# googlegenomics/spark-examples

Hardware: AMD Instinct MI355X
Metric: variants/sec into N×N Gram + PCoA wall-clock, 2504 samples, 1/2/4/8 GPU (higher is better)
Workload: dtype fp4(e2m1)->f32->i32

## Files before the change

spark-examples_amd/csrc/operand.hip:

```cpp
#include <algorithm>
#include <cstring>

#include "pcoa_ctx.h"

using namespace pcoa;

namespace pcoa {

int fold_now(pcoa_ctx* c) {
  const int64_t count = (int64_t)s_count(c);
  if (!c->s64) {
    if (c->s64_spare) {
      c->s64 = c->s64_spare;
      c->s64_spare = nullptr;
    } else {
      HIP_TRY(c, dev_alloc((void**)&c->s64, sizeof(int64_t) * (size_t)count, c->device));
    }
    HIP_TRY(c, hipMemsetAsync(c->s64, 0, sizeof(int64_t) * (size_t)count, c->stream));
  }
  if (!c->is_strip) HIP_TRY(c, launch_symmetrize_i32(c->s32, c->n, c->stream));
  HIP_TRY(c, launch_fold_i32_to_i64(c->s32, c->s64, count, c->stream));
  c->variants_in_s32 = 0;
  c->dirty = false;
  return PCOA_OK;
// ... 8 lines not shown
  return rc;
}

int narrow_s64(pcoa_ctx* c) {
  if (!c->s64 || debug_knobs().no_narrow) return PCOA_OK;
  const int64_t count = (int64_t)s_count(c);
  if (!c->narrow_flag) HIP_TRY(c, dev_alloc((void**)&c->narrow_flag, 16, c->device));
  HIP_TRY(c, hipMemsetAsync(c->narrow_flag, 0, 16, c->stream));
  HIP_TRY(c, launch_narrow_i64_to_i32(c->s64, c->s32, count, c->narrow_flag, c->stream));
  HIP_TRY(c, hipMemcpyAsync(c->hw->coll, c->narrow_flag, 16, hipMemcpyDeviceToHost, c->stream));
  HIP_TRY(c, hipStreamSynchronize(c->stream));
  const int32_t overflow = (int32_t)(c->hw->coll[0] & 0xffffffff);
  const int64_t maxabs = c->hw->coll[1];
  if (overflow) {
    HIP_TRY(c, hipMemsetAsync(c->s32, 0, sizeof(int32_t) * (size_t)count, c->stream));
    return PCOA_OK;
  }
  if ((size_t)count * sizeof(int64_t) <= ((size_t)1 << 30)) {
    c->s64_spare = c->s64;
  } else {
    dev_free(c->s64);
  }
  c->s64 = nullptr;
  c->variants_in_s32 = maxabs;
  c->narrowed += 1;
  return PCOA_OK;
}

void account_gram(pcoa_ctx* c, int64_t cur, int64_t weight) {
  c->gram_launches += 1;
  c->gram_variants += cur;
  c->gram_flops += 2.0 * (double)cur * (double)c->n * (double)c->n;
  c->gram_bytes += 4.0 * (double)cur * (double)c->n + 4.0 * (double)c->n * (double)c->n;
  c->variants_in_s32 += cur * weight;
  c->dirty = true;
  c->strip_centering_set = false;
}

int fold_if_needed(pcoa_ctx* c, int64_t cur) {
  if (c->variants_in_s32 + cur > c->fold_threshold) {
    int rc = fp4_quiesce(c);
    if (rc != PCOA_OK) return rc;
    ScopedTimer t(c, T_FINALIZE);
    return fold_now(c);
  }
  return PCOA_OK;
}

static int64_t fp4_kb_bytes(const pcoa_ctx* c) { return gram_packed_npad(c->n) * (c->op_fmt == 2 ? 4 : 16); }
int64_t kb_of(const pcoa_ctx* c, int64_t nv) {
  const int64_t kb = (nv + 31) / 32;
  return c->op_fmt == 2 ? round_up(kb, 4) : kb;
}
static hipError_t launch_pack_operand(const pcoa_ctx* c, const void* x, int is_u8, int64_t ld, int64_t nv, int8_t* dst, int32_t* flag,
                               hipStream_t s, int64_t kb, int ring_wgs = 0) {
  if (ring_wgs > 0 && c->op_fmt == 2 && !is_u8)
    return launch_pack_kbits_ring(static_cast<const float*>(x), ld, nv, c->n, dst, flag, s, kb / 4, ring_wgs,
                                  8 + 1000 * std::max(0, debug_knobs().kbits_ring_prio));
  if (ring_wgs > 0 && c->op_fmt == 2 && is_u8)
    return launch_pack_kbits_ring_u8(static_cast<const uint8_t*>(x), ld, nv, c->n, dst, flag, s, kb / 4, ring_wgs, 8);
  return c->op_fmt == 2 ? launch_pack_kbits(x, is_u8, ld, nv, c->n, dst, flag, s, kb / 4)
                        : launch_pack_fp4(x, is_u8, ld, nv, c->n, dst, flag, s, kb);
}
static hipError_t launch_bits_operand(const pcoa_ctx* c, const uint32_t* bits, int64_t ld_words, int64_t nv, int8_t* dst, hipStream_t s,
                               int64_t kb) {
  return c->op_fmt == 2 ? launch_transpose_bits_kbits(bits, ld_words, nv, c->n, dst, s, kb / 4)
                        : launch_expand_bits_fp4(bits, ld_words, nv, c->n, dst, s, kb);
}
hipError_t launch_csr_operand(const pcoa_ctx* c, const int32_t* idx, const int64_t* offs, int64_t nv, int64_t offs_base,
                              int8_t* dst, hipStream_t s, int64_t kb) {
  return c->op_fmt == 2 ? launch_densify_csr_kbits(idx, offs, nv, offs_base, dst, c->n, c->err_flag, s, kb / 4)
                        : launch_densify_csr_fp4(idx, offs, nv, offs_base, dst, c->n, c->err_flag, s, kb);
}
static int32_t* fb_flag(pcoa_ctx* c, int b) { return c->fb_flags + 16 * b; }

int64_t fp4_target_kb(const pcoa_ctx* c) {
  const int64_t per_kb = fp4_kb_bytes(c);
  const int64_t by_launch = (c->fb_count == 2) ? kPipeVariants : kBatchVariants;
  return std::max<int64_t>(1, std::min(std::min(c->max_launch, by_launch) / 32, kBatchBytes / per_kb));
}

static int fork_to(pcoa_ctx* c, hipStream_t side) {
  if (side == c->stream) return PCOA_OK;
  if (debug_knobs().fork_lazy != 0) {
    if (hipStreamQuery(c->stream) == hipSuccess) return PCOA_OK;
    (void)hipGetLastError();
  }
  HIP_TRY(c, hipEventRecord(c->ev_fork, c->stream));
  HIP_TRY(c, hipStreamWaitEvent(side, c->ev_fork, 0));
  return PCOA_OK;
}

static int int8_chunk(pcoa_ctx* c, const void* x_chunk, int is_u8, int64_t cur, int64_t ld) {
  int rc = PCOA_OK;
  if ((rc = fp4_quiesce(c)) != PCOA_OK) return rc;
  const int64_t need = (int64_t)gram_packed_workspace_bytes(c->n, cur);
  if ((rc = ensure(c, &c->pack_buf, &c->pack_cap, need)) != PCOA_OK) return rc;
  HIP_TRY(c, hipMemsetAsync(c->err_flag + 1, 0, sizeof(int32_t), c->stream));
  {
    ScopedTimer t(c, T_PACK);
    hipError_t e = is_u8 ? launch_pack_u8_i8(static_cast<const uint8_t*>(x_chunk), ld, cur, c->n, c->pack_buf,
                                             c->err_flag, c->stream)
                         : launch_pack_f32_i8(static_cast<const float*>(x_chunk), ld, cur, c->n, c->pack_buf,
                                              c->err_flag, c->stream);
    if (e != hipSuccess) return hip_fail(c, e, "pack(i8) kernel launch");
    c->pack_launches += 1;
    c->pack_bytes += (is_u8 ? 1.0 : 4.0) * (double)cur * (double)c->n + (double)need;
  }
  HIP_TRY(c, hipMemcpyAsync(&c->hw->mmax, c->err_flag + 1, sizeof(int32_t), hipMemcpyDeviceToHost, c->stream));
  HIP_TRY(c, hipStreamSynchronize(c->stream));
  const int32_t mmax = c->hw->mmax;
// ... 16 lines not shown
}

int fp4_setup(pcoa_ctx* c) {
  if (c->fb_flags) return PCOA_OK;
  HIP_TRY(c, dev_alloc((void**)&c->fb_flags, 256, c->device));
  HIP_TRY(c, hipMemsetAsync(c->fb_flags, 0, 256, c->stream));
  HIP_TRY(c, hipHostMalloc((void**)&c->fb_flags_host, 256, hipHostMallocDefault));
  std::memset(c->fb_flags_host, 0, 256);
  HIP_TRY(c, hipEventCreateWithFlags(&c->ev_fork, hipEventDisableTiming));
  for (auto& b : c->fb) {
    HIP_TRY(c, hipEventCreateWithFlags(&b.packed, hipEventDisableTiming));
    HIP_TRY(c, hipEventCreateWithFlags(&b.consumed, hipEventDisableTiming));
  }
  const DebugKnobs& k = debug_knobs();
  const int ls = gram_lockstep_splitk(c->n, c->num_cu);
  c->lockstep_ok = !c->is_strip && ls > 0 && gram_lockstep_workgroups(c->n, ls) * 5 >= c->num_cu * 4;
  if (k.lockstep == 0) c->lockstep_ok = false;
  if (k.lockstep == 1) c->lockstep_ok = !c->is_strip && ls > 0;
  {
    const int64_t ntile = gram_packed_npad(c->n) / 256;
    const int64_t ntri = c->is_strip ? ntile * ((c->s_cols + 255) / 256 + 1) : ntile * (ntile + 1) / 2;
    c->kbits_mode = (ntri <= 4 * (int64_t)c->num_cu) ? 4 : 0;
    if (k.kbits_mode == 0 || k.kbits_mode == 4) c->kbits_mode = k.kbits_mode;
    if (k.kbits_mode == 5 && c->kbits_mode == 4) c->kbits_mode = 5;
    if (k.kbits_mode == 2 && !c->is_strip && ls > 0) c->kbits_mode = 2;
  }
  const int half = c->num_cu / 2;
  const int lsh = gram_lockstep_splitk(c->n, half);
  bool want = !c->is_strip && c->num_cu >= 64 && lsh > 0 && gram_packed_npad(c->n) >= 5 * 256;
  const int64_t cores_max = k.kbits_coreside_max_npad > 0 ? k.kbits_coreside_max_npad : kCoresideMaxNpad;
  const bool cores_shape = !c->is_strip && c->num_cu >= 64 && c->op_fmt == 2 && k.kbits_coreside != 0 &&
                           gram_packed_npad(c->n) >= 5 * 256 && gram_packed_npad(c->n) <= cores_max;
  want = want || cores_shape;
  if (k.pipeline == 0) want = false;
  if (k.pipeline == 1) want = !c->is_strip && (lsh > 0 || cores_shape);
  if (c->flags & PCOA_FLAG_NO_PIPELINE) want = false;
  if (want) {
    hipError_t e1 = hipStreamCreateWithFlags(&c->pack_stream, hipStreamNonBlocking);
    hipError_t e2 = (e1 == hipSuccess) ? hipStreamCreateWithFlags(&c->gram_stream, hipStreamNonBlocking) : e1;
    if (e1 == hipSuccess && e2 == hipSuccess) {
      c->pipe_ok = true;
      c->pipe_gram_cus = half;
      if (c->op_fmt == 2 && k.kbits_pipe_wgs >= 8 && k.kbits_pipe_wgs <= c->num_cu) c->pipe_gram_cus = k.kbits_pipe_wgs / 8 * 8;
      c->fb_count = 2;
      if (c->op_fmt == 2 && k.kbits_coreside != 0) {
        c->coreside = true;
        c->coreside_mode = (ls > 0 && gram_lockstep_workgroups(c->n, ls) * 5 >= c->num_cu * 4 && k.kbits_mode != 4) ? 2 : c->kbits_mode;
        if (k.kbits_mode == 2 && ls > 0) c->coreside_mode = 2;
        c->pipe_gram_cus = c->num_cu;
        if (k.kbits_pipe_wgs >= 8 && k.kbits_pipe_wgs <= c->num_cu) {
          c->pipe_gram_cus = k.kbits_pipe_wgs / 8 * 8;
          c->coreside_mode = 4;
        }
        c->ring_wgs = (k.kbits_ring_wgs > 0) ? k.kbits_ring_wgs : 2 * c->num_cu;
      }
    } else {
      (void)hipGetLastError();
      if (c->pack_stream) (void)hipStreamDestroy(c->pack_stream);
      c->pack_stream = c->gram_stream = nullptr;
    }
  }
  if (c->op_fmt == 2 && c->kbits_mode != 0) c->fb_count = 2;
  if (!c->pipe_ok && c->lockstep_ok) c->fb_count = 2;
  return PCOA_OK;
}

static int fp4_launch(pcoa_ctx* c, int bi, bool overlapped, int side_kind = 1) {
  pcoa_ctx::Fp4Buf& b = c->fb[bi];
  int rc = (bi == c->fb_active && !c->csr_pending.empty()) ? csr_validate(c) : PCOA_OK;
  if (rc != PCOA_OK) return rc;
  if (b.kb == 0) return PCOA_OK;
  rc = fold_if_needed(c, b.vars);
  if (rc != PCOA_OK) return rc;
  const int64_t per_kb = fp4_kb_bytes(c);
  const int64_t kb_pad = round_up(b.kb, 24);
  const bool side = overlapped && c->pipe_ok;
  hipStream_t gs = side ? c->gram_stream : c->stream;
  if (kb_pad > b.kb)
    HIP_TRY(c, hipMemsetAsync(b.p + b.kb * per_kb, 0, (size_t)((kb_pad - b.kb) * per_kb), b.fill_stream));
  if (gs != b.fill_stream) {
    HIP_TRY(c, hipEventRecord(b.packed, b.fill_stream));
    HIP_TRY(c, hipStreamWaitEvent(gs, b.packed, 0));
  }
  if ((rc = fork_to(c, gs)) != PCOA_OK) return rc;
  const int cus = side ? c->pipe_gram_cus : c->num_cu;
  const int32_t* skip = b.verify ? fb_flag(c, bi) : nullptr;
  {
    ScopedTimer t(c, T_GRAM, gs);
    hipError_t e = hipErrorInvalidValue;
    if (c->op_fmt == 2) {
      const int mode = !side ? c->kbits_mode : !c->coreside ? 4 : (side_kind == 3 ? c->kbits_mode : c->coreside_mode);
      const int w4 = debug_knobs().kbits_w4;
      const bool use_w4 = w4 != 0 && (!(side && c->coreside) || w4 == 2);
      auto launch = [&](int m) {
        return use_w4 ? launch_gram_kbits_w4(b.p, b.kb * 32, c->n, c->s32, cus, gs, m, skip, strip_of(c), debug_knobs().kbits_w4_diag)
                      : launch_gram_kbits(b.p, b.kb * 32, c->n, c->s32, cus, gs, m, skip, strip_of(c));
      };
      e = launch(mode);
      if (e != hipSuccess && mode != 0) {
        (void)hipGetLastError();
        e = launch(0);
      } else if (e == hipSuccess) {
        if (mode == 2) c->lockstep_launches += 1;
        if (mode == 4 || mode == 5) c->evensplit_launches += 1;
        if (side) c->pipeline_launches += 1;
      }
    } else {
// ... 39 lines not shown
    HIP_TRY(c, hipMemsetAsync(fb_flag(c, bi), 0, sizeof(int32_t), c->stream));
    if (redo) {
      c->fp4_fallbacks += (int64_t)b.chunks.size();
      c->i8_streak = 8;
      std::vector<pcoa_ctx::Fp4Chunk> chunks;
      chunks.swap(b.chunks);
      for (const auto& ch : chunks)
        if ((rc = int8_chunk(c, ch.x, ch.is_u8, ch.nv, ch.ld)) != PCOA_OK) break;
    }
  }
  b.chunks.clear();
  return rc;
}

int fp4_quiesce(pcoa_ctx* c) {
  int rc = c->csr_pending.empty() ? PCOA_OK : csr_validate(c);
  for (int bi = 0; bi < 2 && rc == PCOA_OK; ++bi) rc = fp4_resolve(c, bi);
  if (rc != PCOA_OK) return rc;
  for (auto& b : c->fb)
    if (b.kb > 0 && b.fill_stream && b.fill_stream != c->stream) HIP_TRY(c, hipStreamSynchronize(b.fill_stream));
  return PCOA_OK;
}

int fp4_flush(pcoa_ctx* c) {
  int rc = PCOA_OK;
  for (int bi = 0; bi < 2; ++bi)
    if (c->fb[bi].kb > 0 && (rc = fp4_launch(c, bi, false)) != PCOA_OK) return rc;
  return fp4_quiesce(c);
}

int fp4_sync_point(pcoa_ctx* c) {
  int rc = PCOA_OK;
  for (int bi = 0; bi < 2; ++bi)
    if (c->fb[bi].kb > 0 && c->fb[bi].verify && (rc = fp4_launch(c, bi, false)) != PCOA_OK) return rc;
  return fp4_quiesce(c);
}

int fp4_discard(pcoa_ctx* c) {
  if (!c->csr_pending.empty()) {
    const int rc = staging_wait_all(c, c->cs);
    if (rc != PCOA_OK) return rc;
    c->csr_pending.clear();
    if (c->csr_flag) HIP_TRY(c, hipMemsetAsync(c->csr_flag, 0, 16, c->stream));
  }
  for (int bi = 0; bi < 2; ++bi) {
    pcoa_ctx::Fp4Buf& b = c->fb[bi];
    int rc = fp4_resolve(c, bi, false);
    if (rc != PCOA_OK) return rc;
    if (b.kb > 0 && b.fill_stream && b.fill_stream != c->stream) HIP_TRY(c, hipStreamSynchronize(b.fill_stream));
    b.kb = 0;
    b.vars = 0;
    b.chunks.clear();
  }
  return PCOA_OK;
}

int fp4_grow(pcoa_ctx* c, int bi, int64_t kb, int64_t chunk_variants) {
  pcoa_ctx::Fp4Buf& b = c->fb[bi];
  if (b.kb + kb <= b.cap_kb) return PCOA_OK;
  const int64_t per_kb = fp4_kb_bytes(c);
  const int64_t target = std::max(fp4_target_kb(c), kb);
  const int64_t floor_kb = std::max<int64_t>(1, std::min<int64_t>(1024, ((int64_t)256 << 20) / per_kb));
  int64_t want = (chunk_variants >= ((int64_t)1 << 18))
                     ? target
                     : std::min(target, std::max(std::max(b.kb + kb, floor_kb), 2 * b.cap_kb));
  int8_t* fresh = nullptr;
  for (;;) {
    hipError_t e = dev_alloc((void**)&fresh, (size_t)((want + 24) * per_kb), c->device);
    if (e == hipSuccess) break;
    (void)hipGetLastError();
    if (want <= b.kb + kb) return hip_fail(c, e, "allocation of the FP4 operand buffer");
    want = std::max(b.kb + kb, want / 2);
  }
  hipStream_t s = b.fill_stream ? b.fill_stream : c->stream;
  if (b.kb > 0) HIP_TRY(c, hipMemcpyAsync(fresh, b.p, (size_t)(b.kb * per_kb), hipMemcpyDeviceToDevice, s));
  HIP_TRY(c, hipStreamSynchronize(s));
  if (b.launched) HIP_TRY(c, hipEventSynchronize(b.consumed));
  if (b.p) dev_free(b.p);
  b.p = fresh;
  b.cap_kb = want;
  if (c->fb_count == 2 && chunk_variants >= ((int64_t)1 << 18)) {
    pcoa_ctx::Fp4Buf& o = c->fb[bi ^ 1];
    if (o.cap_kb < want && o.kb == 0 && !o.launched) {
      int8_t* twin = nullptr;
      if (dev_alloc((void**)&twin, (size_t)((want + 24) * per_kb), c->device) == hipSuccess) {
        if (o.p) dev_free(o.p);
        o.p = twin;
        o.cap_kb = want;
      } else {
        (void)hipGetLastError();
      }
    }
  }
  return PCOA_OK;
}

int fp4_reserve(pcoa_ctx* c, int64_t kb, int64_t chunk_variants, int side_kind, bool verify, int8_t** dst,
                hipStream_t* stream, int32_t** flag) {
  int rc = fp4_setup(c);
  if (rc != PCOA_OK) return rc;
  pcoa_ctx::Fp4Buf* b = &c->fb[c->fb_active];
  const bool want_side = c->pipe_ok && (side_kind == 1 || (side_kind == 2 && c->coreside) ||
                                        (side_kind == 3 && c->coreside && debug_knobs().bits_pipeline != 0));
  const bool misfit = b->kb > 0 && ((b->fill_stream != c->stream && !want_side) || (verify != b->verify));
  const bool full = b->kb > 0 && b->kb + kb > std::max(fp4_target_kb(c), kb);
  if (misfit || full) {
// ... 188 lines not shown
```

spark-examples_amd/csrc/pack_kbits.hip:

```cpp
#include <cstdlib>
#include <type_traits>

#include "gram_common.h"

namespace pcoa {
namespace {

template <typename T, int VEC, bool NT = false, bool CS = false>
__global__ __launch_bounds__(256) void pack_kbits_kernel(const T* __restrict__ x, int64_t ld, int64_t nv, int n, int npad,
                                                         int64_t nblk, uint32_t* __restrict__ p,
                                                         int32_t* __restrict__ flag) {
  const int lane = threadIdx.x & 63;
  const int wave = __builtin_amdgcn_readfirstlane(threadIdx.x >> 6);
  const int gw = npad >> 8;
  int64_t wid = (int64_t)blockIdx.x * 4 + wave;
  const int c_only = CS ? (int)(wid & 3) : -1;
  if (CS) wid >>= 2;
  const int64_t blk = wid / gw;
  const int g = (int)(wid - blk * gw) * 64 + lane;
  if (blk >= nblk) return;
  const int i0 = g * 4;
  bool bad = false;
  uint32_t badw = 0;
  uint32_t w[4][4];
// ... 30 lines not shown
              is0 = (uint32_t)(raw[t][s] == 0.0f);
            } else {
              const uint32_t b = (raw[t] >> (8 * s)) & 0xffu;
              is1 = (uint32_t)(b == 1u);
              is0 = (uint32_t)(b == 0u);
            }
            const uint32_t live = valid & (uint32_t)(i0 + s < n);
            badw |= live & ((is1 | is0) ^ 1u);
            w[s][c] |= (live & is1) << (h * 16 + t);
          }
        }
      } else {
#pragma unroll
        for (int t = 0; t < 16; ++t) {
          const int64_t row = blk * 128 + c * 32 + h * 16 + t;
          if (row < nv) {
            const T* src = x + row * ld + i0;
#pragma unroll
            for (int s = 0; s < 4; ++s) {
              if (i0 + s < n) {
                const T v = src[s];
                const bool is1 = (v == (T)1);
                bad |= !(is1 || v == (T)0);
                w[s][c] |= (is1 ? 1u : 0u) << (h * 16 + t);
              }
            }
          }
        }
      }
    }
  }
  if constexpr (CS) {
    uint32_t* dst = p + ((size_t)blk * npad + i0) * 4 + c_only;
#pragma unroll
    for (int s = 0; s < 4; ++s)
      dst[4 * s] = c_only == 0 ? w[s][0] : c_only == 1 ? w[s][1] : c_only == 2 ? w[s][2] : w[s][3];
  } else {
    uint4* dst = reinterpret_cast<uint4*>(p + ((size_t)blk * npad + i0) * 4);
#pragma unroll
    for (int s = 0; s < 4; ++s) dst[s] = make_uint4(w[s][0], w[s][1], w[s][2], w[s][3]);
  }
  if (bad || badw) atomicOr(flag, 8);
}

template <int R, int AUX, int C>
__device__ __forceinline__ void ring_rows_kbits(const char* xb, int64_t ldb, int nv, int blk, uint32_t voff, int blkn,
                                                uint32_t voffn, uint8_t* myring, int lane, f32x4_t& a, uint32_t (&w)[4][4],
                                                uint32_t (&bad4)[4]) {
  auto issue = [&](int bq, uint32_t vo, int r, int slot) {
    int row = bq * 128 + r;
    row = row < nv ? row : nv - 1;
    const char* rowp = xb + (int64_t)row * ldb;
    asm volatile("" : "+s"(rowp));
    __builtin_amdgcn_global_load_lds((gptr_t)(rowp + vo), (lptr_t)(myring + slot * 1024), 16, 0, AUX);
  };
#pragma unroll
  for (int t = 0; t < 32; ++t) {
    const int r = C * 32 + t;
    __builtin_amdgcn_s_waitcnt(0xC07F);
    __builtin_amdgcn_sched_barrier(0);
    if (r + R < 128) issue(blk, voff, r + R, t % R);
    else issue(blkn, voffn, r + R - 128, t % R);
    wait_vmcnt<R - 1>();
    __builtin_amdgcn_sched_barrier(0);
    const f32x4_t b = *reinterpret_cast<const f32x4_t*>(myring + ((t + 1) % R) * 1024 + lane * 16);
    __builtin_amdgcn_sched_barrier(0);
    if (blk * 128 + r < nv) {
#pragma unroll
      for (int s2 = 0; s2 < 4; ++s2) {
        const float f = a[s2];
        bad4[s2] |= __float_as_uint(__builtin_fmaf(f, f, -f));
        w[s2][C] |= ((__float_as_uint(f) >> 23) & 1u) << t;
      }
#pragma unroll
      for (int s2 = 0; s2 < 4; ++s2) asm volatile("" : "+v"(w[s2][C]), "+v"(bad4[s2]));
    }
    a = b;
    __builtin_amdgcn_sched_barrier(0);
  }
}

template <int R, int AUX, int PRIO = 0>
__global__ __launch_bounds__(256, 8) void pack_kbits_ring_kernel(const float* __restrict__ x, int64_t ld, int nv, int n, int npad,
                                                                 int n_units, uint32_t* __restrict__ p,
                                                                 int32_t* __restrict__ flag) {
  static_assert(R == 8 || R == 16 || R == 32, "the slot of row t must be a compile-time constant of the 32-row unrolled body");
  extern __shared__ __attribute__((aligned(16))) uint8_t ring_dyn_kbits[];
  if constexpr (PRIO > 0) __builtin_amdgcn_s_setprio(PRIO);
  const int lane = threadIdx.x & 63;
  const int wave = __builtin_amdgcn_readfirstlane(threadIdx.x >> 6);
  const int gw = npad >> 8;
  const int stride = (int)gridDim.x * 4;
  const int stride_b = stride / gw, stride_g = stride - stride_b * gw;
  int u = (int)blockIdx.x * 4 + wave;
  if (u >= n_units) return;
  int blk = u / gw, G = u - blk * gw;
  uint8_t* const myring = ring_dyn_kbits + wave * (R * 1024);
  const char* const xb = reinterpret_cast<const char*>(x);
  const int64_t ldb = ld * 4;
  uint32_t bad = 0;
  auto lane_off = [&](int Gq) -> uint32_t {
    const int col = Gq * 256 + lane * 4;
    return col < ld ? (uint32_t)col * 4u : 0u;
  };
  uint32_t voff = lane_off(G);
#pragma unroll
  for (int t = 0; t < R; ++t) {
    int row = blk * 128 + t;
    row = row < nv ? row : nv - 1;
    __builtin_amdgcn_global_load_lds((gptr_t)(xb + (int64_t)row * ldb + voff), (lptr_t)(myring + t * 1024), 16, 0, AUX);
  }
  wait_vmcnt<R - 1>();
  f32x4_t a = *reinterpret_cast<const f32x4_t*>(myring + lane * 16);
  for (;;) {
    int blkn = blk + stride_b, Gn = G + stride_g;
    if (Gn >= gw) { Gn -= gw; blkn += 1; }
    const bool last = u + stride >= n_units;
    if (last) { blkn = blk; Gn = G; }
    const uint32_t voffn = lane_off(Gn);
    const int col = G * 256 + lane * 4;
    uint32_t w[4][4], bad4[4];
#pragma unroll
    for (int s2 = 0; s2 < 4; ++s2) {
      bad4[s2] = 0;
#pragma unroll
      for (int q = 0; q < 4; ++q) w[s2][q] = 0;
    }
    ring_rows_kbits<R, AUX, 0>(xb, ldb, nv, blk, voff, blkn, voffn, myring, lane, a, w, bad4);
    ring_rows_kbits<R, AUX, 1>(xb, ldb, nv, blk, voff, blkn, voffn, myring, lane, a, w, bad4);
    ring_rows_kbits<R, AUX, 2>(xb, ldb, nv, blk, voff, blkn, voffn, myring, lane, a, w, bad4);
    ring_rows_kbits<R, AUX, 3>(xb, ldb, nv, blk, voff, blkn, voffn, myring, lane, a, w, bad4);
#pragma unroll
    for (int s2 = 0; s2 < 4; ++s2) {
      const uint32_t cm = (col + s2 < n) ? 0xffffffffu : 0u;
      bad |= bad4[s2] & cm;
#pragma unroll
      for (int q = 0; q < 4; ++q) w[s2][q] &= cm;
    }
    uint4* dst = reinterpret_cast<uint4*>(p + ((size_t)blk * npad + col) * 4);
#pragma unroll
    for (int s2 = 0; s2 < 4; ++s2) dst[s2] = make_uint4(w[s2][0], w[s2][1], w[s2][2], w[s2][3]);
    if (last) break;
    u += stride;
    blk = blkn;
    G = Gn;
    voff = voffn;
  }
  wait_vmcnt<0>();
  asm volatile("s_waitcnt lgkmcnt(0)" ::: "memory");
  if (bad) atomicOr(flag, 8);
}

__device__ __forceinline__ uint4 lds_read_b128_asm(uint32_t lds_addr) {
  uint4 v;
  asm volatile("ds_read_b128 %0, %1" : "=v"(v) : "v"(lds_addr) : "memory");
  return v;
}
template <int R, int AUX>
__global__ __launch_bounds__(256, 4) void pack_u8_kbits_ring_kernel(const uint8_t* __restrict__ x, int64_t ld, int nv, int n,
                                                                    int npad, int n_units, uint32_t* __restrict__ p,
                                                                    int32_t* __restrict__ flag) {
  static_assert(R == 8, "the slot of row t must be a compile-time constant of the 8-row unrolled body");
  extern __shared__ __attribute__((aligned(16))) uint8_t ring_dyn_u8[];
  const int lane = threadIdx.x & 63;
  const int wave = __builtin_amdgcn_readfirstlane(threadIdx.x >> 6);
  const int gw = (npad + 1023) >> 10;
  const int stride = (int)gridDim.x * 4;
  const int stride_b = stride / gw, stride_g = stride - stride_b * gw;
  int u = (int)blockIdx.x * 4 + wave;
  if (u >= n_units) return;
  int blk = u / gw, G = u - blk * gw;
  uint8_t* const myring = ring_dyn_u8 + wave * (R * 1024);
  const char* const xb = reinterpret_cast<const char*>(x);
  const int ldi = (int)ld;
  auto lane_off = [&](int Gq, bool& shifted) -> uint32_t {
    const int col = Gq * 1024 + lane * 16;
    shifted = col < ldi && col + 16 > ldi;
    return col + 16 <= ldi ? (uint32_t)col : (col < ldi ? (uint32_t)(ldi - 16) : 0u);
  };
  auto issue = [&](int bq, uint32_t vo, int r, int slot) {
    int row = bq * 128 + r;
    row = row < nv ? row : nv - 1;
    const char* rowp = xb + (int64_t)row * ld;
    asm volatile("" : "+s"(rowp));
    __builtin_amdgcn_global_load_lds((gptr_t)(rowp + vo), (lptr_t)(myring + slot * 1024), 16, 0, AUX);
  };
  bool shifted = false, shiftedn = false;
  uint32_t voff = lane_off(G, shifted);
  uint32_t bad = 0;
#pragma unroll
  for (int t = 0; t < R; ++t) issue(blk, voff, t, t);
  wait_vmcnt<R - 1>();
  const uint32_t lds_lane = (uint32_t)(uintptr_t)(lptr_t)(myring + lane * 16);
  uint4 a = lds_read_b128_asm(lds_lane);
  for (;;) {
    int blkn = blk + stride_b, Gn = G + stride_g;
    if (Gn >= gw) { Gn -= gw; blkn += 1; }
    const bool last = u + stride >= n_units;
    if (last) { blkn = blk; Gn = G; }
    const uint32_t voffn = lane_off(Gn, shiftedn);
    const int col = G * 1024 + lane * 16;
    uint32_t w[16][4], badd[4] = {0, 0, 0, 0};
#pragma unroll
    for (int s2 = 0; s2 < 16; ++s2)
// ... 257 lines not shown
      const int32_t c = cs[i];
      if (c < 0 || c >= n) {
        atomicOr(flag, 1);
        flag[2] = c;
        continue;
      }
      const uint32_t bit = 1u << (row & 31);
      if (atomicOr(&bits[(size_t)c * 4 + (row >> 5)], bit) & bit) atomicOr(flag, 32);
    }
  }
  __syncthreads();
  uint4* dst = reinterpret_cast<uint4*>(p + (size_t)blk * npad * 4);
  for (int i = tid; i < npad; i += THREADS) dst[i] = reinterpret_cast<const uint4*>(bits)[i];
}

}

hipError_t launch_pack_kbits(const void* x, int is_u8, int64_t ld, int64_t nv, int32_t n, int8_t* p, int32_t* flag,
                             hipStream_t stream, int64_t nblk_out) {
  if (nv <= 0) return hipSuccess;
  const int npad = (int)gram_packed_npad(n);
  const int64_t nblk = nblk_out > 0 ? nblk_out : (nv + 127) / 128;
  const int64_t blocks = (nblk * (npad >> 8) + 3) / 4;
  if (blocks > 0x7fffffffLL) return hipErrorInvalidValue;
  uint32_t* pw = reinterpret_cast<uint32_t*>(p);
  const uintptr_t addr = reinterpret_cast<uintptr_t>(x);
  const dim3 grid((unsigned)blocks), block(256);
  if (is_u8) {
    const uint8_t* xs = static_cast<const uint8_t*>(x);
    if (((ld & 7) == 0) && ((addr & 7) == 0)) {
      const int64_t blocks8 = (nblk * (npad >> 3) + 255) / 256;
      if (blocks8 > 0x7fffffffLL) return hipErrorInvalidValue;
      hipLaunchKernelGGL(pack_u8x8_kbits_kernel, dim3((unsigned)blocks8), block, 0, stream, xs, ld, nv, n, npad, nblk, pw,
                         flag);
      return hipGetLastError();
    }
    const bool vec = ((ld & 3) == 0) && ((addr & 3) == 0);
    if (vec) hipLaunchKernelGGL((pack_kbits_kernel<uint8_t, 4>), grid, block, 0, stream, xs, ld, nv, n, npad, nblk, pw, flag);
    else hipLaunchKernelGGL((pack_kbits_kernel<uint8_t, 1>), grid, block, 0, stream, xs, ld, nv, n, npad, nblk, pw, flag);
  } else {
    const bool vec = ((ld & 3) == 0) && ((addr & 15) == 0);
    const float* xs = static_cast<const float*>(x);
    const bool small = nblk * (npad >> 8) < 2560;
    if (vec && small)
      hipLaunchKernelGGL((pack_kbits_kernel<float, 4, true, true>), dim3((unsigned)(nblk * (npad >> 8))), block, 0, stream, xs, ld, nv,
                         n, npad, nblk, pw, flag);
    else if (vec) hipLaunchKernelGGL((pack_kbits_kernel<float, 4, true>), grid, block, 0, stream, xs, ld, nv, n, npad, nblk, pw, flag);
    else hipLaunchKernelGGL((pack_kbits_kernel<float, 1>), grid, block, 0, stream, xs, ld, nv, n, npad, nblk, pw, flag);
  }
  return hipGetLastError();
}

hipError_t launch_pack_kbits_ring(const float* x, int64_t ld, int64_t nv, int32_t n, int8_t* p, int32_t* flag,
                                  hipStream_t stream, int64_t nblk_out, int wgs, int ring) {
  if (nv <= 0) return hipSuccess;
  if (!pack_fp4_ring_ok(x, ld) || nv > 0x3fffffffLL) return hipErrorInvalidValue;
  const int npad = (int)gram_packed_npad(n);
  const int64_t nblk = nblk_out > 0 ? nblk_out : (nv + 127) / 128;
  const int64_t units = nblk * (npad >> 8);
  if (units > 0x3fffffffLL) return hipErrorInvalidValue;
  uint32_t* pw = reinterpret_cast<uint32_t*>(p);
  const int64_t most = (units + 3) / 4;
  const dim3 grid((unsigned)(wgs > 0 && wgs < most ? wgs : most)), block(256);
#define PCOA_RINGK(R_, AUX_, PRIO_)                                                                                        \
  hipLaunchKernelGGL((pack_kbits_ring_kernel<R_, AUX_, PRIO_>), grid, block, 4 * R_ * 1024, stream, x, ld, (int)nv, n, npad, \
                     (int)units, pw, flag)
  ring %= 10000;
#ifdef PCOA_EXPERIMENTS
  if (ring >= 5000) {
    switch (ring - 5000) {
      case 1: PCOA_RINGK(8, 1, 0); break;
      case 3: PCOA_RINGK(8, 3, 0); break;
      case 16: PCOA_RINGK(8, 16, 0); break;
      case 17: PCOA_RINGK(8, 17, 0); break;
      case 18: PCOA_RINGK(8, 18, 0); break;
      default: PCOA_RINGK(8, 0, 0); break;
    }
    return hipGetLastError();
  }
  const int R = ring % 100, nt = (ring / 100) % 10, prio = ring / 1000;
#define PCOA_RINGK2(R_)                                                       \
  do {                                                                        \
    if (nt && prio) PCOA_RINGK(R_, 2, 3);                                     \
    else if (nt) PCOA_RINGK(R_, 2, 0);                                        \
    else if (prio) PCOA_RINGK(R_, 0, 3);                                      \
    else PCOA_RINGK(R_, 0, 0);                                                \
  } while (0)
  if (R == 8) PCOA_RINGK2(8);
  else if (R == 32) PCOA_RINGK2(32);
  else PCOA_RINGK2(16);
#undef PCOA_RINGK2
#else
  if ((ring / 100) % 10) PCOA_RINGK(8, 2, 0);
  else if (ring / 1000) PCOA_RINGK(8, 0, 3);
  else PCOA_RINGK(8, 0, 0);
#endif
#undef PCOA_RINGK
  return hipGetLastError();
}

bool pack_u8_ring_ok(const void* x, int64_t ld) {
  return ((ld & 7) == 0) && ld >= 16 && ((reinterpret_cast<uintptr_t>(x) & 7) == 0);
}
hipError_t launch_pack_kbits_ring_u8(const uint8_t* x, int64_t ld, int64_t nv, int32_t n, int8_t* p, int32_t* flag,
                                     hipStream_t stream, int64_t nblk_out, int wgs, int ring) {
  if (nv <= 0) return hipSuccess;
  if (!pack_u8_ring_ok(x, ld) || nv > 0x3fffffffLL || ld > 0x3fffffffLL) return hipErrorInvalidValue;
  const int npad = (int)gram_packed_npad(n);
  const int64_t nblk = nblk_out > 0 ? nblk_out : (nv + 127) / 128;
  const int64_t units = nblk * ((npad + 1023) >> 10);
  if (units > 0x3fffffffLL) return hipErrorInvalidValue;
  uint32_t* pw = reinterpret_cast<uint32_t*>(p);
  const int64_t most = (units + 3) / 4;
  const dim3 grid((unsigned)(wgs > 0 && wgs < most ? wgs : most)), block(256);
  if ((ring / 100) % 10)
    hipLaunchKernelGGL((pack_u8_kbits_ring_kernel<8, 2>), grid, block, 32 << 10, stream, x, ld, (int)nv, n, npad, (int)units, pw, flag);
  else
    hipLaunchKernelGGL((pack_u8_kbits_ring_kernel<8, 0>), grid, block, 32 << 10, stream, x, ld, (int)nv, n, npad, (int)units, pw, flag);
  return hipGetLastError();
// ... 62 lines not shown
```

spark-examples_amd/csrc/pcoa_ctx.h:

```cpp
#pragma once

#include <algorithm>
#include <chrono>

#include "pcoa_internal.h"

enum TimeCat { T_GRAM = 0, T_DENSIFY, T_SYNTH, T_FINALIZE, T_CENTER, T_TRIDIAG, T_EIG, T_BACK, T_PACK, T_LANCZOS, T_ALLREDUCE, T_NCAT };

struct EventPair {
  hipEvent_t a, b;
  int cat;
};

struct StagingRing {
  struct Slot {
    void* dev[2] = {nullptr, nullptr};
    size_t dev_bytes[2] = {0, 0};
    void* pin[2] = {nullptr, nullptr};
    size_t pin_bytes[2] = {0, 0};
    hipEvent_t copied = nullptr, freed = nullptr;
    bool used = false;
  };
  Slot slot[2];
  int next = 0;
// ... 40 lines not shown
  int64_t csr_offs_cap = 0;
  StagingRing cs;
  hipStream_t csr_stream = nullptr;
  int32_t* csr_flag = nullptr;
  int32_t* csr_flag_host = nullptr;
  struct CsrPending { const int32_t* idx; const int64_t* offs; int64_t nv; int64_t kb; bool device; };
  std::vector<CsrPending> csr_pending;
  double csr_stage_s = 0, csr_wait_s = 0;
  int64_t csr_fast_chunks = 0, csr_redo_chunks = 0;
  StagingRing bs;
  uint32_t* thr_dev = nullptr;
  int64_t thr_cap = 0;
  int32_t* sample_pop = nullptr;
  std::vector<int32_t> pop_offsets_dev;
  StagingRing ts;
  int64_t* xfer = nullptr;
  size_t xfer_bytes = 0;
  int32_t* narrow_flag = nullptr;
  int64_t reduce_i32_calls = 0, narrowed = 0, allreduce_calls = 0;
  int32_t comm_ranks = 0, allreduce_int32 = 0, matvec_form = 0, lanczos_block_steps = 0;
  int64_t* coll = nullptr;
  int8_t* pack_buf = nullptr;
  int64_t pack_cap = 0;
  bool use_i8 = true;
  int packed_mode = 0;
  int op_fmt = 2;
  int64_t fp4_fallbacks = 0;
  int i8_streak = 0;
  struct Fp4Chunk { const void* x; int is_u8; int64_t nv, ld; };
  struct Fp4Buf {
    int8_t* p = nullptr;
    int64_t cap_kb = 0;
    int64_t kb = 0, vars = 0;
    hipStream_t fill_stream = nullptr;
    hipEvent_t packed = nullptr, consumed = nullptr;
    bool launched = false;
    bool verify = false;
    int64_t launched_vars = 0;
    std::vector<Fp4Chunk> chunks;
  };
  Fp4Buf fb[2];
  int fb_count = 1, fb_active = 0;
  int32_t* fb_flags = nullptr;
  int32_t* fb_flags_host = nullptr;
  bool pipe_ok = false;
  int pipe_gram_cus = 0;
  hipStream_t pack_stream = nullptr, gram_stream = nullptr;
  hipEvent_t ev_fork = nullptr;
  bool lockstep_ok = false;
  int kbits_mode = 4;
  bool coreside = false;
  int coreside_mode = 4;
  int ring_wgs = 0;
  int64_t lockstep_launches = 0, pipeline_launches = 0, evensplit_launches = 0;
  int64_t pack_chunk = (int64_t)1 << 20;
  int64_t pack_launches = 0;
  double pack_bytes = 0;

  bool ws_ready = false;
  pcoa::EigWorkspace ws{};
  double* row_sums = nullptr;
  double* colmean = nullptr;
  double* stats = nullptr;
  int32_t* nz = nullptr;
  double* out_dev = nullptr;
  int32_t kmax = 0;
  double* lanczos_ws = nullptr;
  double* sym_part = nullptr;
  int64_t sym_part_cap = 0;
  int64_t lanczos_cap = 0;
  int32_t eig_method = 0;
  int32_t eig_dense_form = 0;
  int32_t lanczos_steps = 0;

  std::vector<EventPair> pending;
  std::vector<hipEvent_t> pool;
  double tsec[T_NCAT] = {0};
  int64_t gram_launches = 0;
  int64_t gram_variants = 0;
  double gram_flops = 0, gram_bytes = 0;
  double compute_total = 0;
  int gram_kind = 1;
  int64_t max_launch = (int64_t)1 << 24;
  int64_t fold_threshold = (int64_t)1 << 30;
};

#define HIP_TRY(ctx, expr)                                     \
  do {                                                         \
    hipError_t _e = (expr);                                    \
    if (_e != hipSuccess) return hip_fail((ctx), _e, #expr);   \
  } while (0)

#define CHECK_CTX(ctx)                                                      \
  do {                                                                      \
    if (!(ctx)) return fail(nullptr, PCOA_ERR_INVALID_ARG, "ctx is NULL");  \
    hipError_t _e = hipSetDevice((ctx)->device);                            \
    if (_e != hipSuccess) return hip_fail((ctx), _e, "hipSetDevice");       \
  } while (0)

namespace pcoa {

constexpr int64_t KB_I8 = 16;
constexpr int64_t kMaxLaunchVariants = (int64_t)1 << 24;
constexpr int64_t kFoldThreshold = (int64_t)1 << 30;
constexpr int64_t kBatchVariants = (int64_t)1 << 22;
constexpr int64_t kBatchBytes = (int64_t)6 << 30;
constexpr int64_t kPipeVariants = (int64_t)1 << 20;
constexpr int64_t kCoresideMaxNpad = 16384;

inline int64_t round_up(int64_t v, int64_t m) { return (v + m - 1) / m * m; }
inline double wall_now() { return std::chrono::duration<double>(std::chrono::steady_clock::now().time_since_epoch()).count(); }
inline size_t s_count(const pcoa_ctx* c) { return (size_t)c->n * (size_t)c->s_cols; }
inline GramStrip strip_of(const pcoa_ctx* c) {
  GramStrip st;
  if (c->is_strip) { st.col0 = c->strip_col0; st.cols = c->s_cols; }
  return st;
}

hipError_t dev_alloc(void** out, size_t bytes, int device);
void dev_free(void* p);
int regrow(pcoa_ctx* c, void** buf, size_t bytes, bool sync_ctx_stream);

int fail(pcoa_ctx* c, int code, const std::string& msg);
int hip_fail(pcoa_ctx* c, hipError_t e, const char* what);
hipEvent_t get_event(pcoa_ctx* c);
void drain_events(pcoa_ctx* c, bool wait);

int fold_now(pcoa_ctx* c);
int ensure_xfer(pcoa_ctx* c, size_t bytes);
int narrow_s64(pcoa_ctx* c);
void account_gram(pcoa_ctx* c, int64_t cur, int64_t weight = 1);
int fold_if_needed(pcoa_ctx* c, int64_t cur);
int64_t kb_of(const pcoa_ctx* c, int64_t nv);
int64_t fp4_target_kb(const pcoa_ctx* c);
hipError_t launch_csr_operand(const pcoa_ctx* c, const int32_t* idx, const int64_t* offs, int64_t nv, int64_t offs_base,
                              int8_t* dst, hipStream_t s, int64_t kb);
int fp4_setup(pcoa_ctx* c);
int fp4_quiesce(pcoa_ctx* c);
int fp4_flush(pcoa_ctx* c);
int fp4_sync_point(pcoa_ctx* c);
int fp4_discard(pcoa_ctx* c);
int fp4_grow(pcoa_ctx* c, int bi, int64_t kb, int64_t chunk_variants);
int fp4_reserve(pcoa_ctx* c, int64_t kb, int64_t chunk_variants, int side_kind, bool verify, int8_t** dst,
                hipStream_t* stream, int32_t** flag);
void fp4_commit(pcoa_ctx* c, int64_t kb, int64_t vars);
int gram_device(pcoa_ctx* c, const void* x_dev, int is_u8, int64_t nv, int64_t ld, bool can_defer);
int gram_device_bits(pcoa_ctx* c, const uint32_t* bits_dev, int64_t nv, int64_t ld_words, bool can_defer);
int check_device_flags(pcoa_ctx* c);
int finalize_impl(pcoa_ctx* c);

int csr_validate(pcoa_ctx* c);
int staging_wait_all(pcoa_ctx* c, StagingRing& r);
void staging_destroy(StagingRing& r);

int ensure_workspace(pcoa_ctx* c, int32_t k);
int ensure_b(pcoa_ctx* c);

struct ScopedTimer {
  pcoa_ctx* c;
  EventPair p;
  hipStream_t s;
// ... 30 lines not shown
```

spark-examples_amd/csrc/pcoa_internal.h:

```cpp
#ifndef PCOA_INTERNAL_H_
#define PCOA_INTERNAL_H_

#include <hip/hip_runtime.h>
#include <stdint.h>

#include <functional>
#include <string>
#include <vector>

#include "pcoa.h"

namespace pcoa {

constexpr int kWave = 64;
constexpr int kNumXcd = 8;

struct DebugKnobs {
  int gram_kernel = -1;
  int64_t pack_chunk = 0;
  int64_t max_launch = 0;
  int64_t fold_threshold = 0;
  int pipeline = -1;
  int explicit_center = 0;
  int lanczos_first_check = 0;
// ... 33 lines not shown
  int32_t* flag;
  const float* zeros;
  int num_cu;
  hipStream_t stream;
};
hipError_t launch_gram_f32(const GramLaunch& g, int* splitk_out);

struct GramStrip {
  int col0 = 0, cols = 0;
  int cb0 = 0;
};

int64_t gram_packed_npad(int32_t n);
int64_t gram_packed_kb_pad_i8(int64_t nv);
size_t gram_packed_workspace_bytes(int32_t n, int64_t nv);
int64_t gram_kb_pad(int64_t nv, int fmt);
int gram_lockstep_splitk(int32_t n, int cus);
int gram_lockstep_workgroups(int32_t n, int splitk);

hipError_t launch_pack_f32_i8(const float* x, int64_t ld, int64_t nv, int32_t n, int8_t* p, int32_t* flag,
                              hipStream_t stream);
hipError_t launch_pack_u8_i8(const uint8_t* x, int64_t ld, int64_t nv, int32_t n, int8_t* p, int32_t* flag,
                             hipStream_t stream);
hipError_t launch_densify_csr_i8(const int32_t* idx_dev, const int64_t* offs_dev, int64_t nv, int64_t offs_base,
                                 int8_t* p, int32_t n, int32_t* flag, hipStream_t stream);
hipError_t launch_densify_csr_fp4(const int32_t* idx_dev, const int64_t* offs_dev, int64_t nv, int64_t offs_base,
                                  int8_t* p, int32_t n, int32_t* flag, hipStream_t stream, int64_t nkb_out);
hipError_t launch_expand_bits_fp4(const uint32_t* bits, int64_t ld_words, int64_t nv, int32_t n, int8_t* p,
                                  hipStream_t stream, int64_t nkb_out = 0);
hipError_t launch_pack_fp4(const void* x, int is_u8, int64_t ld, int64_t nv, int32_t n, int8_t* p, int32_t* flag,
                           hipStream_t stream, int64_t nkb_out = 0);
bool pack_fp4_ring_ok(const void* x, int64_t ld);
#ifdef PCOA_EXPERIMENTS
hipError_t launch_pack_fp4_ring(const float* x, int64_t ld, int64_t nv, int32_t n, int8_t* p, int32_t* flag,
                                hipStream_t stream, int64_t nkb_out, int wgs, int nt);
#endif

hipError_t launch_gram_packed(const int8_t* p, int fmt, int64_t nv, int32_t n, int32_t* s32, int num_cu,
                              hipStream_t stream, int* splitk_out, const int32_t* skip = nullptr,
                              GramStrip strip = GramStrip{});
hipError_t launch_gram_packed_lockstep(const int8_t* p, int fmt, int64_t nv, int32_t n, int32_t* s32, int num_cu,
                                       hipStream_t stream, const int32_t* skip = nullptr);
#ifdef PCOA_EXPERIMENTS
extern int g_lockstep_map;
#endif

hipError_t launch_pack_kbits(const void* x, int is_u8, int64_t ld, int64_t nv, int32_t n, int8_t* p, int32_t* flag,
                             hipStream_t stream, int64_t nblk_out);
hipError_t launch_transpose_bits_kbits(const uint32_t* bits, int64_t ld_words, int64_t nv, int32_t n, int8_t* p,
                                       hipStream_t stream, int64_t nblk_out);
hipError_t launch_densify_csr_kbits(const int32_t* idx_dev, const int64_t* offs_dev, int64_t nv, int64_t offs_base,
                                    int8_t* p, int32_t n, int32_t* flag, hipStream_t stream, int64_t nblk_out);
hipError_t launch_pack_kbits_ring(const float* x, int64_t ld, int64_t nv, int32_t n, int8_t* p, int32_t* flag,
                                  hipStream_t stream, int64_t nblk_out, int wgs, int ring);
bool pack_u8_ring_ok(const void* x, int64_t ld);
hipError_t launch_pack_kbits_ring_u8(const uint8_t* x, int64_t ld, int64_t nv, int32_t n, int8_t* p, int32_t* flag,
                                     hipStream_t stream, int64_t nblk_out, int wgs, int ring);

hipError_t launch_gram_kbits(const int8_t* p, int64_t nv, int32_t n, int32_t* s32, int num_cu, hipStream_t stream, int mode,
                             const int32_t* skip = nullptr, GramStrip strip = GramStrip{});
hipError_t launch_gram_kbits_w4(const int8_t* p, int64_t nv, int32_t n, int32_t* s32, int num_cu, hipStream_t stream, int mode,
                                const int32_t* skip = nullptr, GramStrip strip = GramStrip{}, int wdiag = -1);

hipError_t launch_densify_csr(const int32_t* idx_dev, const int64_t* offs_dev, int64_t v0, int64_t nv,
                              int64_t offs_base, float* x_dev, int64_t ld, int32_t n, int32_t* err_flag_dev,
                              hipStream_t stream);
hipError_t launch_delay_us(hipStream_t stream, int microseconds);
hipError_t launch_symmetrize_i32(int32_t* s32, int32_t n, hipStream_t stream);
hipError_t launch_fold_i32_to_i64(int32_t* s32, int64_t* s64, int64_t count, hipStream_t stream);
hipError_t launch_export_i64(const int32_t* s32, const int64_t* s64_or_null, int64_t* dst, int64_t count,
                             hipStream_t stream);
hipError_t launch_plink_bed_to_bits(const uint8_t* bed, int64_t row_bytes, int64_t nv, int32_t n, int64_t words, int ref_a1,
                                    uint32_t* bits, hipStream_t stream);
hipError_t launch_add_i64(int64_t* dst, const int64_t* src, int64_t count, hipStream_t stream);
hipError_t launch_add_i32(int32_t* dst, const int32_t* src, int64_t count, hipStream_t stream);
hipError_t launch_narrow_i64_to_i32(const int64_t* s64, int32_t* s32, int64_t count, int32_t* flag, hipStream_t stream);
hipError_t launch_synth_fill_f32(uint64_t seed, const uint32_t* thresholds_dev, const int32_t* sample_pop_dev,
                                 int32_t n_pops, int64_t first_variant, int64_t nv, int32_t n, float* x_dev,
                                 int64_t ld, hipStream_t stream);

hipError_t launch_synth_kbits(uint64_t seed, const uint32_t* thresholds_dev, const int32_t* sample_pop_dev, int32_t n_pops,
                              int64_t first_variant, int64_t nv, int32_t n, int32_t npad, int8_t* p, int64_t nblk_out,
                              hipStream_t stream);

hipError_t launch_col_means(const double* row_sums, int32_t n, double* cm, hipStream_t stream);
hipError_t launch_center(const int32_t* s32, const int64_t* s64_or_null, int32_t n, double* row_sums,
                         double* stats, int32_t* nz, double* b, hipStream_t stream, bool row_sums_done = false);

int64_t strip_ws_doubles(int32_t n, int32_t cols);
hipError_t launch_strip_col_sums(const int32_t* s32, const int64_t* s64_or_null, int32_t n, int32_t cols, double* ws,
                                 hipStream_t stream);
hipError_t launch_strip_matvec(const int32_t* s32, const int64_t* s64_or_null, int32_t n, int32_t col0, int32_t cols,
                               const double* v, const double* means, double matrix_mean, double* ws, hipStream_t stream);
hipError_t launch_strip_col_sums_to(const int32_t* s32, const int64_t* s64_or_null, int32_t n, int32_t cols, double* ws,
                                    int64_t* out_i64, double* out_f64, hipStream_t stream);
hipError_t launch_strip_matvec_to(const int32_t* s32, const int64_t* s64_or_null, int32_t n, int32_t col0, int32_t cols,
                                  const double* v, const double* means, double matrix_mean, double* ws, double* y_out,
                                  hipStream_t stream);

int64_t project_ws_doubles(int32_t n_ref, int32_t cols, int32_t k);
int project_chunk(int32_t remaining);
hipError_t launch_project(const int32_t* s32, const int64_t* s64_or_null, int32_t n_ref, int32_t cols, const double* colsum,
                          const double* means, double matrix_mean, const double* u, int32_t k, const double* lam, double* ws,
                          double* out, hipStream_t stream);

constexpr int32_t EIG_FORM_FUSED = 1;
constexpr int32_t EIG_FORM_FUSED_BIG_LDS = 2;
// ... 50 lines not shown
```

Baseline: 517.9 million.

## Use atomic ticket queue for ring pack work distribution and size grid by idle CUs

After: 490.3 million. 0.947x the previous value.

```diff
diff --git a/spark-examples_amd/csrc/operand.hip b/spark-examples_amd/csrc/operand.hip
--- a/spark-examples_amd/csrc/operand.hip
+++ b/spark-examples_amd/csrc/operand.hip
@@ -84,11 +84,18 @@
   const int64_t kb = (nv + 31) / 32;
   return c->op_fmt == 2 ? round_up(kb, 4) : kb;
 }
-static hipError_t launch_pack_operand(const pcoa_ctx* c, const void* x, int is_u8, int64_t ld, int64_t nv, int8_t* dst, int32_t* flag,
+static hipError_t launch_pack_operand(pcoa_ctx* c, const void* x, int is_u8, int64_t ld, int64_t nv, int8_t* dst, int32_t* flag,
                                hipStream_t s, int64_t kb, int ring_wgs = 0) {
-  if (ring_wgs > 0 && c->op_fmt == 2 && !is_u8)
+  if (ring_wgs > 0 && c->op_fmt == 2 && !is_u8) {
+    uint32_t* tickets = reinterpret_cast<uint32_t*>(c->fb_flags + 48);
+    if (c->ring_ticket_base >= 0x80000000u) {
+      hipError_t e = hipMemsetAsync(tickets, 0, sizeof(uint32_t), s);
+      if (e != hipSuccess) return e;
+      c->ring_ticket_base = 0;
+    }
     return launch_pack_kbits_ring(static_cast<const float*>(x), ld, nv, c->n, dst, flag, s, kb / 4, ring_wgs,
-                                  8 + 1000 * std::max(0, debug_knobs().kbits_ring_prio));
+                                  8 + 1000 * std::max(0, debug_knobs().kbits_ring_prio), tickets, &c->ring_ticket_base);
+  }
   if (ring_wgs > 0 && c->op_fmt == 2 && is_u8)
     return launch_pack_kbits_ring_u8(static_cast<const uint8_t*>(x), ld, nv, c->n, dst, flag, s, kb / 4, ring_wgs, 8);
   return c->op_fmt == 2 ? launch_pack_kbits(x, is_u8, ld, nv, c->n, dst, flag, s, kb / 4)
@@ -211,7 +218,8 @@
           c->pipe_gram_cus = k.kbits_pipe_wgs / 8 * 8;
           c->coreside_mode = 4;
         }
-        c->ring_wgs = (k.kbits_ring_wgs > 0) ? k.kbits_ring_wgs : 2 * c->num_cu;
+        const int busy = std::min<int>(c->num_cu, c->coreside_mode == 2 ? gram_lockstep_workgroups(c->n, ls) : c->pipe_gram_cus);
+        c->ring_wgs = (k.kbits_ring_wgs > 0) ? k.kbits_ring_wgs : 2 * busy + kRingWgsFreeCu * (c->num_cu - busy);
       }
     } else {
       (void)hipGetLastError();
@@ -357,6 +365,10 @@
     b.vars = 0;
     b.chunks.clear();
   }
+  if (c->fb_flags && c->ring_ticket_base != 0) {
+    HIP_TRY(c, hipMemsetAsync(c->fb_flags + 48, 0, sizeof(uint32_t), c->stream));
+    c->ring_ticket_base = 0;
+  }
   return PCOA_OK;
 }
 
diff --git a/spark-examples_amd/csrc/pack_kbits.hip b/spark-examples_amd/csrc/pack_kbits.hip
--- a/spark-examples_amd/csrc/pack_kbits.hip
+++ b/spark-examples_amd/csrc/pack_kbits.hip
@@ -106,7 +106,9 @@
     row = row < nv ? row : nv - 1;
     const char* rowp = xb + (int64_t)row * ldb;
     asm volatile("" : "+s"(rowp));
-    __builtin_amdgcn_global_load_lds((gptr_t)(rowp + vo), (lptr_t)(myring + slot * 1024), 16, 0, AUX);
+    uint32_t ring = (uint32_t)(uintptr_t)(lptr_t)myring;
+    asm volatile("" : "+s"(ring));
+    __builtin_amdgcn_global_load_lds((gptr_t)(rowp + vo), (lptr_t)(uintptr_t)(ring + slot * 1024), 16, 0, AUX);
   };
 #pragma unroll
   for (int t = 0; t < 32; ++t) {
@@ -134,28 +136,47 @@
   }
 }
 
-template <int R, int AUX, int PRIO = 0>
-__global__ __launch_bounds__(256, 8) void pack_kbits_ring_kernel(const float* __restrict__ x, int64_t ld, int nv, int n, int npad,
-                                                                 int n_units, uint32_t* __restrict__ p,
-                                                                 int32_t* __restrict__ flag) {
+__device__ __forceinline__ uint32_t ring_ticket_draw(uint32_t* tickets, int lane) {
+  uint32_t tv = 0;
+  if (lane == 0) {
+    uint32_t zoff;
+    asm volatile("v_mov_b32 %0, 1\n\tv_mov_b32 %1, 0\n\tglobal_atomic_add %0, %1, %0, %2 sc0"
+                 : "=&v"(tv), "=&v"(zoff) : "s"(tickets) : "memory");
+  }
+  return tv;
+}
+__device__ __forceinline__ uint32_t ring_ticket_unit(uint32_t tv, uint32_t base) {
+  uint32_t t;
+  asm volatile("v_readfirstlane_b32 %0, %1" : "=s"(t) : "v"(tv));
+  return t - base;
+}
+
+template <int R, int AUX, int PRIO, bool QUEUE>
+__device__ __forceinline__ void ring_kbits_body(const float* __restrict__ x, int64_t ld, int nv, int n, int npad, int n_units,
+                                                uint32_t* __restrict__ p, int32_t* __restrict__ flag, uint32_t* tickets,
+                                                uint32_t base) {
   static_assert(R == 8 || R == 16 || R == 32, "the slot of row t must be a compile-time constant of the 32-row unrolled body");
   extern __shared__ __attribute__((aligned(16))) uint8_t ring_dyn_kbits[];
   if constexpr (PRIO > 0) __builtin_amdgcn_s_setprio(PRIO);
   const int lane = threadIdx.x & 63;
   const int wave = __builtin_amdgcn_readfirstlane(threadIdx.x >> 6);
-  const int gw = npad >> 8;
-  const int stride = (int)gridDim.x * 4;
-  const int stride_b = stride / gw, stride_g = stride - stride_b * gw;
-  int u = (int)blockIdx.x * 4 + wave;
-  if (u >= n_units) return;
-  int blk = u / gw, G = u - blk * gw;
+  const uint32_t gw = (uint32_t)npad >> 8;
+  const uint32_t stride = gridDim.x * 4u;
+  uint32_t u = blockIdx.x * 4u + (uint32_t)wave;
+  if constexpr (QUEUE) {
+    const uint32_t tv = ring_ticket_draw(tickets, lane);
+    wait_vmcnt<0>();
+    u = ring_ticket_unit(tv, base);
+  }
+  if (u >= (uint32_t)n_units) return;
+  int blk = (int)(u / gw), G = (int)(u - (uint32_t)blk * gw);
   uint8_t* const myring = ring_dyn_kbits + wave * (R * 1024);
   const char* const xb = reinterpret_cast<const char*>(x);
   const int64_t ldb = ld * 4;
   uint32_t bad = 0;
   auto lane_off = [&](int Gq) -> uint32_t {
-    const int col = Gq * 256 + lane * 4;
-    return col < ld ? (uint32_t)col * 4u : 0u;
+    const uint32_t off = (uint32_t)(Gq * 256 + lane * 4) * 4u;
+    return (int64_t)off < ldb ? off : 0u;
   };
   uint32_t voff = lane_off(G);
 #pragma unroll
@@ -167,11 +188,8 @@
   wait_vmcnt<R - 1>();
   f32x4_t a = *reinterpret_cast<const f32x4_t*>(myring + lane * 16);
   for (;;) {
-    int blkn = blk + stride_b, Gn = G + stride_g;
-    if (Gn >= gw) { Gn -= gw; blkn += 1; }
-    const bool last = u + stride >= n_units;
-    if (last) { blkn = blk; Gn = G; }
-    const uint32_t voffn = lane_off(Gn);
+    uint32_t tv = 0;
+    if constexpr (QUEUE) tv = ring_ticket_draw(tickets, lane);
     const int col = G * 256 + lane * 4;
     uint32_t w[4][4], bad4[4];
 #pragma unroll
@@ -180,9 +198,18 @@
 #pragma unroll
       for (int q = 0; q < 4; ++q) w[s2][q] = 0;
     }
-    ring_rows_kbits<R, AUX, 0>(xb, ldb, nv, blk, voff, blkn, voffn, myring, lane, a, w, bad4);
-    ring_rows_kbits<R, AUX, 1>(xb, ldb, nv, blk, voff, blkn, voffn, myring, lane, a, w, bad4);
-    ring_rows_kbits<R, AUX, 2>(xb, ldb, nv, blk, voff, blkn, voffn, myring, lane, a, w, bad4);
+    ring_rows_kbits<R, AUX, 0>(xb, ldb, nv, blk, voff, blk, voff, myring, lane, a, w, bad4);
+    ring_rows_kbits<R, AUX, 1>(xb, ldb, nv, blk, voff, blk, voff, myring, lane, a, w, bad4);
+    ring_rows_kbits<R, AUX, 2>(xb, ldb, nv, blk, voff, blk, voff, myring, lane, a, w, bad4);
+    uint32_t un = u + stride;
+    if constexpr (QUEUE) un = ring_ticket_unit(tv, base);
+    const bool last = un >= (uint32_t)n_units;
+    int blkn = blk, Gn = G;
+    if (!last) {
+      blkn = (int)(un / gw);
+      Gn = (int)(un - (uint32_t)blkn * gw);
+    }
+    const uint32_t voffn = lane_off(Gn);
     ring_rows_kbits<R, AUX, 3>(xb, ldb, nv, blk, voff, blkn, voffn, myring, lane, a, w, bad4);
 #pragma unroll
     for (int s2 = 0; s2 < 4; ++s2) {
@@ -191,11 +218,11 @@
 #pragma unroll
       for (int q = 0; q < 4; ++q) w[s2][q] &= cm;
     }
-    uint4* dst = reinterpret_cast<uint4*>(p + ((size_t)blk * npad + col) * 4);
+    uint4* dst = reinterpret_cast<uint4*>(p + ((size_t)blk * (gw << 8) + col) * 4);
 #pragma unroll
     for (int s2 = 0; s2 < 4; ++s2) dst[s2] = make_uint4(w[s2][0], w[s2][1], w[s2][2], w[s2][3]);
     if (last) break;
-    u += stride;
+    u = un;
     blk = blkn;
     G = Gn;
     voff = voffn;
@@ -204,6 +231,22 @@
   asm volatile("s_waitcnt lgkmcnt(0)" ::: "memory");
   if (bad) atomicOr(flag, 8);
 }
+
+template <int R, int AUX, int PRIO = 0>
+__global__ __launch_bounds__(256, 8) void pack_kbits_ring_kernel(const float* __restrict__ x, int64_t ld, int nv, int n, int npad,
+                                                                 int n_units, uint32_t* __restrict__ p,
+                                                                 int32_t* __restrict__ flag, uint32_t* tickets,
+                                                                 uint32_t base) {
+  ring_kbits_body<R, AUX, PRIO, true>(x, ld, nv, n, npad, n_units, p, flag, tickets, base);
+}
+#ifdef PCOA_EXPERIMENTS
+template <int R, int AUX, int PRIO = 0>
+__global__ __launch_bounds__(256, 8) void pack_kbits_ring_static_kernel(const float* __restrict__ x, int64_t ld, int nv, int n,
+                                                                        int npad, int n_units, uint32_t* __restrict__ p,
+                                                                        int32_t* __restrict__ flag) {
+  ring_kbits_body<R, AUX, PRIO, false>(x, ld, nv, n, npad, n_units, p, flag, nullptr, 0u);
+}
+#endif
 
 __device__ __forceinline__ uint4 lds_read_b128_asm(uint32_t lds_addr) {
   uint4 v;
@@ -567,7 +610,8 @@
 }
 
 hipError_t launch_pack_kbits_ring(const float* x, int64_t ld, int64_t nv, int32_t n, int8_t* p, int32_t* flag,
-                                  hipStream_t stream, int64_t nblk_out, int wgs, int ring) {
+                                  hipStream_t stream, int64_t nblk_out, int wgs, int ring, uint32_t* tickets,
+                                  uint32_t* ticket_base) {
   if (nv <= 0) return hipSuccess;
   if (!pack_fp4_ring_ok(x, ld) || nv > 0x3fffffffLL) return hipErrorInvalidValue;
   const int npad = (int)gram_packed_npad(n);
@@ -577,9 +621,25 @@
   uint32_t* pw = reinterpret_cast<uint32_t*>(p);
   const int64_t most = (units + 3) / 4;
   const dim3 grid((unsigned)(wgs > 0 && wgs < most ? wgs : most)), block(256);
+  if (tickets && !ticket_base) return hipErrorInvalidValue;
+  const uint32_t base = tickets ? *ticket_base : 0u;
+  if (tickets) *ticket_base = base + (uint32_t)units + 4u * grid.x;
+#ifdef PCOA_EXPERIMENTS
+#define PCOA_RINGK(R_, AUX_, PRIO_)                                                                                          \
+  do {                                                                                                                       \
+    if (tickets)                                                                                                             \
+      hipLaunchKernelGGL((pack_kbits_ring_kernel<R_, AUX_, PRIO_>), grid, block, 4 * R_ * 1024, stream, x, ld, (int)nv, n,    \
+                         npad, (int)units, pw, flag, tickets, base);                                                         \
+    else                                                                                                                     \
+      hipLaunchKernelGGL((pack_kbits_ring_static_kernel<R_, AUX_, PRIO_>), grid, block, 4 * R_ * 1024, stream, x, ld, (int)nv, \
+                         n, npad, (int)units, pw, flag);                                                                     \
+  } while (0)
+#else
+  if (!tickets) return hipErrorInvalidValue;
 #define PCOA_RINGK(R_, AUX_, PRIO_)                                                                                        \
   hipLaunchKernelGGL((pack_kbits_ring_kernel<R_, AUX_, PRIO_>), grid, block, 4 * R_ * 1024, stream, x, ld, (int)nv, n, npad, \
-                     (int)units, pw, flag)
+                     (int)units, pw, flag, tickets, base)
+#endif
   ring %= 10000;
 #ifdef PCOA_EXPERIMENTS
   if (ring >= 5000) {
diff --git a/spark-examples_amd/csrc/pcoa_ctx.h b/spark-examples_amd/csrc/pcoa_ctx.h
--- a/spark-examples_amd/csrc/pcoa_ctx.h
+++ b/spark-examples_amd/csrc/pcoa_ctx.h
@@ -116,6 +116,7 @@
   bool coreside = false;
   int coreside_mode = 4;
   int ring_wgs = 0;
+  uint32_t ring_ticket_base = 0;
   int64_t lockstep_launches = 0, pipeline_launches = 0, evensplit_launches = 0;
   int64_t pack_chunk = (int64_t)1 << 20;
   int64_t pack_launches = 0;
@@ -171,6 +172,7 @@
 constexpr int64_t kBatchBytes = (int64_t)6 << 30;
 constexpr int64_t kPipeVariants = (int64_t)1 << 20;
 constexpr int64_t kCoresideMaxNpad = 16384;
+constexpr int kRingWgsFreeCu = 2;
 
 inline int64_t round_up(int64_t v, int64_t m) { return (v + m - 1) / m * m; }
 inline double wall_now() { return std::chrono::duration<double>(std::chrono::steady_clock::now().time_since_epoch()).count(); }
diff --git a/spark-examples_amd/csrc/pcoa_internal.h b/spark-examples_amd/csrc/pcoa_internal.h
--- a/spark-examples_amd/csrc/pcoa_internal.h
+++ b/spark-examples_amd/csrc/pcoa_internal.h
@@ -109,7 +109,8 @@
 hipError_t launch_densify_csr_kbits(const int32_t* idx_dev, const int64_t* offs_dev, int64_t nv, int64_t offs_base,
                                     int8_t* p, int32_t n, int32_t* flag, hipStream_t stream, int64_t nblk_out);
 hipError_t launch_pack_kbits_ring(const float* x, int64_t ld, int64_t nv, int32_t n, int8_t* p, int32_t* flag,
-                                  hipStream_t stream, int64_t nblk_out, int wgs, int ring);
+                                  hipStream_t stream, int64_t nblk_out, int wgs, int ring, uint32_t* tickets = nullptr,
+                                  uint32_t* ticket_base = nullptr);
 bool pack_u8_ring_ok(const void* x, int64_t ld);
 hipError_t launch_pack_kbits_ring_u8(const uint8_t* x, int64_t ld, int64_t nv, int32_t n, int8_t* p, int32_t* flag,
                                      hipStream_t stream, int64_t nblk_out, int wgs, int ring);
```
